# aniketntnu/WordDiffusion

Measured on AMD Instinct MI355X. Metric: denoised 64x256 word images/sec (1000-step DDPM), whole job, higher is better.
Workload: dtype bf16x3; 1 GPU; BASELINE configs[1]: batch 64 per GPU of 64x256 crops = [64,4,8,32] latents, 1000-step DDPM (999 executed steps), base unet.py UNetModel (320 ch, mult (1,1), 4 heads, 339 writers), random-init synthetic weights; variant=base, batch_per_gpu=64, noise_steps=1000, executed_steps_per_image=999, precision=split-bf16 MFMA x3, fp32 accumulate (<=1e-4 of the fp32 reference), output_finite=True

## Files before the change

include/wdiff_hip.h:

```cpp
#ifndef WDIFF_HIP_H
#define WDIFF_HIP_H

#include <stdint.h>

#ifdef __cplusplus
extern "C" {
#endif

#define WD_OK 0
#define WD_EINVAL (-1)
#define WD_ELAUNCH (-2)
#define WD_ESTATE (-3)

#define WD_ACT_NONE 0
#define WD_ACT_SILU 1
#define WD_ACT_GEGLU 2

typedef uint16_t wd_bf16;

#define WD_MAX_KSPLIT 64

typedef struct wd_src {
    const wd_bf16* hi;
    const wd_bf16* lo;
// ... 122 lines not shown
int wd_gemm_auto_ksplit(int m, int n, int ktot, int64_t ws_floats);
int wd_gemm_args_bytes(void);
int wd_gemm_experimental(void);

int wd_gn_nchunk(int hw);
int wd_gn_stats(const float* x, int ld, int batch, int hw, int c, int cpg, double* part, void* stream);
int wd_gn_fold_chunks(const double* part, int batch, int nchunk, int ngroups, double* out, void* stream);

int wd_gn_apply(const float* x, int ld, int batch, int hw, int c, int cpg, const double* part, int nchunk, int part_cpg,
                const float* gamma, const float* beta, float eps, int silu,
                wd_bf16* out_hi, wd_bf16* out_lo, int out_ld, int c_off,
                wd_bf16* raw_hi, wd_bf16* raw_lo, void* stream);

int wd_gn_apply2(const float* xa, int lda, int ca, const double* part_a, int nchunk_a, int part_cpg_a, int c_off_a,
                 const float* xb, int ldb, int cb, const double* part_b, int nchunk_b, int part_cpg_b, int c_off_b,
                 int batch, int hw, int cpg, const float* gamma, const float* beta, float eps, int silu,
                 wd_bf16* out_hi, wd_bf16* out_lo, int out_ld, wd_bf16* raw_hi, wd_bf16* raw_lo, const int32_t* perm_a, void* stream);

int wd_gn_conv3x3_few_supported(int c, int w, int oc);
int wd_gn_conv3x3_few(const float* x, int ld, int batch, int h, int w, int c, int cpg, const double* part, int nchunk, int part_cpg,
                      const float* gamma, const float* beta, float eps, int silu, const float* weight, const float* bias, int oc,
                      float* out, void* stream);

int wd_layernorm(const float* x, int ld, int rows, int c, const float* gamma, const float* beta, float eps,
                 wd_bf16* out_hi, wd_bf16* out_lo, int out_ld, void* stream);

int wd_split(const float* x, int ld, int rows, int c, int silu, wd_bf16* out_hi, wd_bf16* out_lo, int out_ld,
             void* stream);

int wd_attention(const float* q, int ldq, const float* k, int ldk, const float* v, int ldv,
                 int batch, int heads, int nq, int nk, int d, float scale,
                 float* out_f32, wd_bf16* out_hi, wd_bf16* out_lo, int out_ld, int out_rows, int out_row0,
                 void* stream);

int64_t wd_attention_packed_elems(int batch, int heads, int nk, int d);
int wd_attention_pack_kv(const float* k, int ldk, const float* v, int ldv, int batch, int heads, int nk, int d,
                         wd_bf16* img, void* stream);
int wd_attention_packed(const float* q, int ldq, const wd_bf16* img, int batch, int heads, int nq, int nk, int d,
                        float scale, float* out_f32, wd_bf16* out_hi, wd_bf16* out_lo, int out_ld, int out_rows,
                        int out_row0, void* stream);

int wd_timestep_embedding(const int64_t* t, int batch, const float* freqs, int half,
                          wd_bf16* out_hi, wd_bf16* out_lo, int out_ld, void* stream);

int wd_xattn_supported(int c, int heads, int L);
int wd_xattn_fold(const float* k, int ldk, const float* v, int ldv, int batch, int heads, int L, int d, float scale,
// ... 168 lines not shown
```

worddiffusion_amd/_native.py:

```python
from __future__ import annotations

import ctypes as C
import os
import re

_HERE = os.path.dirname(os.path.abspath(__file__))
LIB_PATH = os.environ.get("WDIFF_LIB") or os.path.join(_HERE, "libwdiff_hip.so")
HEADER_PATH = os.path.join(os.path.dirname(_HERE), "include", "wdiff_hip.h")

WD_OK, WD_EINVAL, WD_ELAUNCH, WD_ESTATE = 0, -1, -2, -3
ACT_NONE, ACT_SILU, ACT_GEGLU = 0, 1, 2
NCLASS = 13
CLASS_NAMES = ("gemm", "gn_stats", "gn_apply", "layernorm", "attention", "other", "gemm_other_tiles", "gemm_splitk_reduce",
               "gemm_two_per_cu", "gemm_weights_to_registers", "feed_forward_fused", "weight_gradient", "gemm_small_maps_whole_k")

_vp = C.c_void_p
_i = C.c_int
_f = C.c_float
_u64 = C.c_uint64


class WdSrc(C.Structure):
    _fields_ = [("hi", _vp), ("lo", _vp), ("gather", _vp), ("ld", C.c_int32), ("c", C.c_int32),
                ("ntaps", C.c_int32), ("hw_src", C.c_int32)]
# ... 42 lines not shown

_SIGS = {
    "wd_gemm": (_i, [C.POINTER(WdGemmArgs), _vp]),
    "wd_gemm_check": (_i, [C.POINTER(WdGemmArgs), C.POINTER(WdGemmArgs)]),
    "wd_dw": (_i, [C.POINTER(WdDwArgs), _vp]),
    "wd_dw_supported": (_i, [_i, _i, _i, _i, _i]),
    "wd_dw_slices": (_i, [_i, _i, _i, _i]),
    "wd_dw_args_bytes": (_i, []),
    "wd_dw_group": (_i, [C.POINTER(WdDwArgs), _vp, _vp, _i, _vp]),
    "wd_dw_group_slices": (_i, [_i, _i, _i, _i, _i]),
    "wd_dw_item_bytes": (_i, []),
    "wd_gemm_auto_ksplit": (_i, [_i, _i, _i, C.c_int64]),
    "wd_gemm_pack_w": (_i, [_vp, _vp, _i, _i, _vp, _vp, _vp]),
    "wd_ff_fused": (_i, [C.POINTER(WdFfArgs), _vp]),
    "wd_ff_supported": (_i, [_i, _i]),
    "wd_ff_args_bytes": (_i, []),
    "wd_gemm_args_bytes": (_i, []),
    "wd_gemm_experimental": (_i, []),
    "wd_gn_nchunk": (_i, [_i]),
    "wd_gn_stats": (_i, [_vp, _i, _i, _i, _i, _i, _vp, _vp]),
    "wd_gn_fold_chunks": (_i, [_vp, _i, _i, _i, _vp, _vp]),
    "wd_gn_conv3x3_few_supported": (_i, [_i, _i, _i]),
    "wd_gn_conv3x3_few": (_i, [_vp, _i, _i, _i, _i, _i, _i, _vp, _i, _i, _vp, _vp, _f, _i, _vp, _vp, _i, _vp, _vp]),
    "wd_gn_apply": (_i, [_vp, _i, _i, _i, _i, _i, _vp, _i, _i, _vp, _vp, _f, _i, _vp, _vp, _i, _i, _vp, _vp, _vp]),
    "wd_gn_apply2": (_i, [_vp, _i, _i, _vp, _i, _i, _i, _vp, _i, _i, _vp, _i, _i, _i, _i, _i, _i, _vp, _vp, _f, _i, _vp, _vp, _i, _vp,
                          _vp, _vp, _vp]),
    "wd_layernorm": (_i, [_vp, _i, _i, _i, _vp, _vp, _f, _vp, _vp, _i, _vp]),
    "wd_split": (_i, [_vp, _i, _i, _i, _i, _vp, _vp, _i, _vp]),
    "wd_attention": (_i, [_vp, _i, _vp, _i, _vp, _i, _i, _i, _i, _i, _i, _f, _vp, _vp, _vp, _i, _i, _i, _vp]),
    "wd_attention_packed_elems": (C.c_int64, [_i, _i, _i, _i]),
    "wd_attention_pack_kv": (_i, [_vp, _i, _vp, _i, _i, _i, _i, _i, _vp, _vp]),
    "wd_attention_packed": (_i, [_vp, _i, _vp, _i, _i, _i, _i, _i, _f, _vp, _vp, _vp, _i, _i, _i, _vp]),
    "wd_timestep_embedding": (_i, [_vp, _i, _vp, _i, _vp, _vp, _i, _vp]),
    "wd_embed_tokens": (_i, [_vp, _i, _i, _i, _vp, _i, _i, _vp, _vp, _vp, _i, _vp]),
    "wd_im2col3x3": (_i, [_vp, _i, _i, _i, _i, _vp, _vp, _i, _vp]),
    "wd_nchw_to_tokens": (_i, [_vp, _i, _i, _i, _vp, _i, _vp]),
    "wd_tokens_to_nchw": (_i, [_vp, _i, _i, _i, _i, _vp, _vp]),
    "wd_ddpm_step": (_i, [_vp, _vp, _i, _i, _vp, _vp, _vp, _vp, _vp, _u64, _u64, _vp]),
    "wd_advance_timestep": (_i, [_vp, _i, _vp, _i, _vp]),
    "wd_randn": (_i, [_vp, _i, _i, _u64, _u64, C.c_uint32, _vp]),
    "wd_noise_images": (_i, [_vp, _vp, _vp, _vp, _vp, _i, _i, _vp, _vp]),
    "wd_copy2d": (_i, [_vp, C.c_int64, _vp, C.c_int64, C.c_int64, C.c_int64, _vp]),
    "wd_ema_update": (_i, [_vp, _vp, C.c_int64, C.c_double, _vp]),
    "wd_adamw_table_entry_bytes": (_i, []),
    "wd_adamw_chunk": (_i, []),
    "wd_adamw_multi": (_i, [_vp, _i, C.c_int64, C.c_double, C.c_double, C.c_double, C.c_double, C.c_double, C.c_int64, _i,
# ... 100 lines not shown
```

worddiffusion_amd/csrc/wd_norm.hip:

```cpp
#include "wd_common.h"

namespace {

constexpr int GN_TOK = 32;

__global__ void gn_stats_kernel(const float* __restrict__ x, int ld, int hw, int c, int cpg, int nchunk,
                                double* __restrict__ part) {
    extern __shared__ __attribute__((aligned(16))) char smem[];
    float* s_sum = reinterpret_cast<float*>(smem);
    float* s_sq = s_sum + 2 * c;
    const int b = blockIdx.y, j = blockIdx.x;
    const int cx = threadIdx.x * 4;
    const int t0 = j * GN_TOK, t1 = min(hw, t0 + GN_TOK);
    if (cx < c) {
        float4 s = make_float4(0, 0, 0, 0), q = make_float4(0, 0, 0, 0);
        const float* base = x + ((long)b * hw) * ld + cx;
        for (int t = t0 + threadIdx.y; t < t1; t += 2) {
            const float4 v = *reinterpret_cast<const float4*>(base + (long)t * ld);
            s.x += v.x; s.y += v.y; s.z += v.z; s.w += v.w;
            q.x += v.x * v.x; q.y += v.y * v.y; q.z += v.z * v.z; q.w += v.w * v.w;
        }
        *reinterpret_cast<float4*>(s_sum + threadIdx.y * c + cx) = s;
        *reinterpret_cast<float4*>(s_sq + threadIdx.y * c + cx) = q;
    }
    __syncthreads();
    const int ng = c / cpg;
    const int tid = threadIdx.y * blockDim.x + threadIdx.x;
// ... 19 lines not shown
};

__global__ void gn_apply_kernel(const GnSrc s0, const GnSrc s1, int hw, int cpg, const float* __restrict__ gamma,
                                const float* __restrict__ beta, float eps, int silu, wd_bf16* __restrict__ out_hi,
                                wd_bf16* __restrict__ out_lo, int out_ld, wd_bf16* __restrict__ raw_hi,
                                wd_bf16* __restrict__ raw_lo) {
    const GnSrc& sr = blockIdx.z ? s1 : s0;
    const float* __restrict__ x = sr.x;
    const double* __restrict__ part = sr.part;
    const int ld = sr.ld, c = sr.c, nchunk = sr.nchunk, part_cpg = sr.part_cpg, c_off = sr.c_off;
    __shared__ float s_mean[32], s_rstd[32];
    const int b = blockIdx.y;
    const int ng = c / cpg;
    if (threadIdx.x < ng) {
        const int ratio = cpg / part_cpg, ngs = c / part_cpg;
        double ds = 0.0, dq = 0.0;
        for (int j = 0; j < nchunk; ++j) {
            const double* p = part + (((long)b * nchunk + j) * ngs + threadIdx.x * ratio) * 2;
            for (int k = 0; k < ratio; ++k) {
                ds += p[2 * k];
                dq += p[2 * k + 1];
            }
        }
        const double n = (double)hw * cpg;
        const double mean = ds / n;
        double var = dq / n - mean * mean;
        if (var < 0.0) var = 0.0;
        s_mean[threadIdx.x] = (float)mean;
        s_rstd[threadIdx.x] = (float)(1.0 / sqrt(var + (double)eps));
    }
    __syncthreads();
    const int c4 = c >> 2;
    const int t0 = blockIdx.x * AP_TOK, nt = min(AP_TOK, hw - t0);
    if (c4 <= 256) {
        const int rpp = 256 / c4;
        const int tl = threadIdx.x / c4, cx = (threadIdx.x - tl * c4) * 4;
        if (tl >= rpp) return;
        float sc[4], sh[4];
#pragma unroll
        for (int j = 0; j < 4; ++j) {
            const int g = (cx + j) / cpg;
            sc[j] = s_rstd[g] * gamma[c_off + cx + j];
            sh[j] = beta[c_off + cx + j] - s_mean[g] * sc[j];
        }
        for (int t = tl; t < nt; t += rpp) {
            const long row = (long)b * hw + t0 + t;
            const long srow = sr.perm ? (long)b * hw + sr.perm[t0 + t] : row;
            const float4 v = *reinterpret_cast<const float4*>(x + srow * ld + cx);
            float4 y = make_float4(v.x * sc[0] + sh[0], v.y * sc[1] + sh[1], v.z * sc[2] + sh[2], v.w * sc[3] + sh[3]);
            if (silu) {
                y.x = wd_silu(y.x); y.y = wd_silu(y.y); y.z = wd_silu(y.z); y.w = wd_silu(y.w);
            }
            uint2 h, l;
            wd_split4(y, h, l);
            const long o = row * out_ld + c_off + cx;
            *reinterpret_cast<uint2*>(out_hi + o) = h;
            if (out_lo) *reinterpret_cast<uint2*>(out_lo + o) = l;
            if (raw_hi) {
                wd_split4(v, h, l);
                *reinterpret_cast<uint2*>(raw_hi + o) = h;
                if (raw_lo) *reinterpret_cast<uint2*>(raw_lo + o) = l;
            }
        }
        return;
    }
    const int total = nt * c4;
    for (int i = threadIdx.x; i < total; i += blockDim.x) {
        const int t = i / c4, cx = (i - t * c4) * 4;
        const long row = (long)b * hw + t0 + t;
        const long srow = sr.perm ? (long)b * hw + sr.perm[t0 + t] : row;
        const float4 v = *reinterpret_cast<const float4*>(x + srow * ld + cx);
        float4 y;
        {
            const int g = cx / cpg, g1 = (cx + 1) / cpg, g2 = (cx + 2) / cpg, g3 = (cx + 3) / cpg;
            const float4 ga = *reinterpret_cast<const float4*>(gamma + c_off + cx);
// ... 204 lines not shown
    *reinterpret_cast<float4*>(s_red + ((long)cg * PXL + pl) * 4) = acc;
    __syncthreads();
    for (int i = tid; i < W * oc; i += 256) {
        const int o = i / W, px = i - o * W;
        float v = bias ? bias[o] : 0.f;
        for (int g = 0; g < CG; ++g) v += s_red[((long)g * PXL + px) * 4 + o];
        out[(((long)b * oc + o) * H + y) * W + px] = v;
    }
}

__global__ void __launch_bounds__(256) gn_fold_chunks_kernel(const double* __restrict__ part, int nchunk, int ng2,
                                                            double* __restrict__ out) {
    __shared__ double red[4][64];
    const int col = threadIdx.x & 63, lane = threadIdx.x >> 6;
    const long b = blockIdx.x;
    double acc = 0.0;
    if (col < ng2)
        for (int j = lane; j < nchunk; j += 4) acc += part[(b * nchunk + j) * ng2 + col];
    red[lane][col] = acc;
    __syncthreads();
    if (lane == 0 && col < ng2) out[b * ng2 + col] = (red[0][col] + red[1][col]) + (red[2][col] + red[3][col]);
}

}

extern "C" int wd_gn_nchunk(int hw) { return (hw + GN_TOK - 1) / GN_TOK; }

extern "C" int wd_gn_fold_chunks(const double* part, int batch, int nchunk, int ngroups, double* out, void* stream) {
    if (!part || !out || batch <= 0 || nchunk <= 0 || ngroups <= 0 || ngroups > 32) return WD_EINVAL;
    hipStream_t st = reinterpret_cast<hipStream_t>(stream);
    WdLaunchScope scope(WD_CLS_GNSTATS, st);
    hipLaunchKernelGGL(gn_fold_chunks_kernel, dim3(batch), dim3(256), 0, st, part, nchunk, 2 * ngroups, out);
    return wd_check_launch();
}

extern "C" int wd_gn_stats(const float* x, int ld, int batch, int hw, int c, int cpg, double* part, void* stream) {
    if (!x || !part || batch <= 0 || hw <= 0 || c <= 0 || cpg <= 0) return WD_EINVAL;
    if (c % 4 || ld % 4 || c % cpg || c / cpg > 256 || c > 4096) return WD_EINVAL;
    hipStream_t st = reinterpret_cast<hipStream_t>(stream);
    const int nchunk = wd_gn_nchunk(hw);
    const int bx = 64 * ((c / 4 + 63) / 64);
    if (bx * 2 > 1024) return WD_EINVAL;
    WdLaunchScope scope(WD_CLS_GNSTATS, st);
    hipLaunchKernelGGL(gn_stats_kernel, dim3(nchunk, batch), dim3(bx, 2), 4 * c * sizeof(float), st, x, ld, hw, c, cpg,
                       nchunk, part);
    return wd_check_launch();
// ... 35 lines not shown

extern "C" int wd_gn_conv3x3_few_supported(int c, int w, int oc) {
    return c > 0 && c % GC_CH == 0 && w > 0 && w <= 64 && oc >= 1 && oc <= 4 &&
           (size_t)(9 * GC_CH * 4 + gn_conv_tile_floats(w)) * sizeof(float) <= 64 * 1024;
}

extern "C" int wd_gn_conv3x3_few(const float* x, int ld, int batch, int h, int w, int c, int cpg, const double* part, int nchunk,
                                 int part_cpg, const float* gamma, const float* beta, float eps, int silu, const float* weight,
                                 const float* bias, int oc, float* out, void* stream) {
    if (!x || !part || !gamma || !beta || !weight || !out || batch <= 0 || h <= 0 || nchunk <= 0 || part_cpg <= 0) return WD_EINVAL;
    if (!wd_gn_conv3x3_few_supported(c, w, oc) || ld % 4 || cpg <= 0 || c % cpg || c / cpg > 32 || cpg % part_cpg) return WD_EINVAL;
    hipStream_t st = reinterpret_cast<hipStream_t>(stream);
    const size_t smem = (size_t)(9 * GC_CH * 4 + gn_conv_tile_floats(w)) * sizeof(float);
    WdLaunchScope scope(WD_CLS_OTHER, st);
    if (w <= 32)
        hipLaunchKernelGGL(gn_conv_few_kernel<32>, dim3(batch, h), dim3(256), smem, st, x, ld, h, w, c, cpg, nchunk, part_cpg, part,
                           gamma, beta, eps, silu, weight, bias, oc, out);
    else
        hipLaunchKernelGGL(gn_conv_few_kernel<64>, dim3(batch, h), dim3(256), smem, st, x, ld, h, w, c, cpg, nchunk, part_cpg, part,
                           gamma, beta, eps, silu, weight, bias, oc, out);
    return wd_check_launch();
}

extern "C" int wd_layernorm(const float* x, int ld, int rows, int c, const float* gamma, const float* beta, float eps,
                            wd_bf16* out_hi, wd_bf16* out_lo, int out_ld, void* stream) {
    if (!x || !gamma || !beta || !out_hi || rows <= 0 || c <= 0) return WD_EINVAL;
    if (c % 4 || ld % 4 || out_ld % 4 || c > 64 * 4 * LN_MAX4) return WD_EINVAL;
    hipStream_t st = reinterpret_cast<hipStream_t>(stream);
    WdLaunchScope scope(WD_CLS_LN, st);
    hipLaunchKernelGGL(layernorm_kernel, dim3((rows + 3) / 4), dim3(256), 0, st, x, ld, rows, c, gamma, beta, eps,
                       out_hi, out_lo, out_ld);
    return wd_check_launch();
}

extern "C" int wd_split(const float* x, int ld, int rows, int c, int silu, wd_bf16* out_hi, wd_bf16* out_lo, int out_ld,
                        void* stream) {
    if (!x || !out_hi || rows <= 0 || c <= 0 || c % 4 || ld % 4 || out_ld % 4) return WD_EINVAL;
    hipStream_t st = reinterpret_cast<hipStream_t>(stream);
    const long total = (long)rows * (c / 4);
    const int grid = (int)((total + 255) / 256 < 2048 ? (total + 255) / 256 : 2048);
    WdLaunchScope scope(WD_CLS_OTHER, st);
    hipLaunchKernelGGL(split_kernel, dim3(grid), dim3(256), 0, st, x, ld, rows, c, silu, out_hi, out_lo, out_ld);
    return wd_check_launch();
}
```

worddiffusion_amd/engine.py:

```python
from __future__ import annotations

import ctypes as C
import math
import os
from typing import Dict, List, Optional, Tuple

import numpy as np
import torch

from . import _native as N
from .layers import (DownsampleParams, ResBlockParams, SpatialTransformerParams, UpsampleParams)


def conv_gather_table(h: int, w: int, mode: str) -> Tuple[np.ndarray, int, int]:
    if mode == "same":
        ho, wo = h, w
    elif mode == "down":
        ho, wo = (h + 2 - 3) // 2 + 1, (w + 2 - 3) // 2 + 1
    elif mode == "up":
        ho, wo = 2 * h, 2 * w
    else:
        raise ValueError(mode)
    yy, xx = np.meshgrid(np.arange(ho), np.arange(wo), indexing="ij")
    tab = np.full((9, ho * wo), -1, dtype=np.int32)
# ... 192 lines not shown
                assert p.is_cuda and p.dtype == torch.float32 and p.is_contiguous(), name
                if mode == 2:
                    hi, lo, ld, ntc = d.data_ptr() + 4 * col_off, 0, 0, 1
                    nch = (n + vchunk - 1) // vchunk
                else:
                    ld = r.cols
                    o = 2 * (row_off * ld + col_off)
                    hi, lo = d[0].data_ptr() + o, d[1].data_ptr() + o
                    ntc = (c + tile - 1) // tile
                    nch = (((npad if mode == 1 else n) + tile - 1) // tile) * ntc
                recs.append(struct.pack("<QQQQiiiiiiiiqii", p.data_ptr(), p2.data_ptr() if p2 is not None else 0, hi, lo, n, c, t,
                                        mode, npad, ld, g, ntc, c0, 0, 0))
                c0 += nch
                if frag is not None and name in frag and self.frag_ok(r):
                    f = frag[name]
                    recs.append(struct.pack("<QQQQiiiiiiiiqii", p.data_ptr(), 0, f[0].data_ptr(), f[1].data_ptr(), n, c, t, 3, 0,
                                            r.rows, g, ntc, c0, row_off, col_off))
                    c0 += nch
        raw = torch.frombuffer(bytearray(b"".join(recs)), dtype=torch.uint8).to(dev)
        return raw, c0, len(recs)


class Act:
    __slots__ = ("t", "c", "h", "w", "stats", "prod", "perm")

    def __init__(self, t, c, h, w, stats=None, prod=None, perm=None):
        self.t, self.c, self.h, self.w = t, c, h, w
        self.perm = perm
        self.stats = stats
        self.prod = prod


class Plan:
    def __init__(self):
        self.cond: List[tuple] = []
        self.step: List[tuple] = []
        self.keep: List[object] = []
        self.out: Optional[torch.Tensor] = None

    @staticmethod
    def _run(ops, stream):
        for fn, args, what in ops:
            rc = fn(*args, stream)
            if rc != 0:
                N.check(rc, what)

    def run_cond(self, stream):
        self._run(self.cond, stream)

    def run_film(self, stream):
# ... 24 lines not shown
        self._pack = None
        self._w: Dict[str, torch.Tensor] = {}
        self._w3: Dict[str, torch.Tensor] = {}
        self._w3_meta: Dict[str, tuple] = {}
        self._wf: Dict[str, torch.Tensor] = {}
        self.use_wdirect = os.environ.get("WDIFF_GEMM_WDIRECT", "1") != "0"
        self.use_up_phases = os.environ.get("WDIFF_UPSAMPLE_PHASES", "1") != "0"
        self._derived: Dict[str, tuple] = {}
        self.use_smallmap = os.environ.get("WDIFF_GEMM_SMALLMAP", "1") != "0"
        self.fuse_ff = os.environ.get("WDIFF_FUSE_FF", "1") != "0"
        self.fuse_proj = os.environ.get("WDIFF_FUSE_PROJ", "1") != "0"
        self.fuse_ln = os.environ.get("WDIFF_FUSE_LN", "1") != "0"
        self.fuse_gn_in = int(os.environ.get("WDIFF_FUSE_GN_IN", "1"))
        self.use_slab = os.environ.get("WDIFF_SLAB", "0") != "0"
        self.fuse_stats = os.environ.get("WDIFF_FUSE_STATS", "1") != "0"
        self.fuse_xattn = os.environ.get("WDIFF_FUSE_XATTN", "1") != "0"
        self.use_conv3 = os.environ.get("WDIFF_CONV3", "0") != "0"
        if (self.use_slab or self.use_conv3) and not self.lib.wd_gemm_experimental():
            raise N.NativeError("WDIFF_SLAB / WDIFF_CONV3 need a library built with WDIFF_EXPERIMENTAL=1 "
                                "(python -m worddiffusion_amd.build --force)")
        self.fuse_xattn_pair = os.environ.get("WDIFF_FUSE_XATTN_PAIR", "1") != "0"
        self.fuse_st = os.environ.get("WDIFF_FUSE_ST", "1") != "0"
        self.fuse_out = os.environ.get("WDIFF_FUSE_OUT", "1") != "0"
        self.pack_kv = os.environ.get("WDIFF_PACK_KV", "1") != "0"
        self.fuse_gn2 = os.environ.get("WDIFF_FUSE_GN2", "1") != "0"
        self.fuse_gn = os.environ.get("WDIFF_FUSE_GN", "1") != "0"
        self.fuse_split = os.environ.get("WDIFF_FUSE_SPLIT", "1") != "0"
        self._plans: Dict[tuple, Plan] = {}
        self._tabs: Dict[tuple, torch.Tensor] = {}
        self._tab_np: Dict[int, np.ndarray] = {}
        self._same_w: Dict[int, int] = {}
        self._down_w: Dict[int, int] = {}
        self._ws = None
        self.device = None

    def set_precision(self, mode: str):
        npass = {"bf16x3": 3, "fp32": 3, "bf16": 1}[mode]
        if npass != self.npass:
            self.npass = npass
            self._plans.clear()

    def _recipes(self) -> "RecipeBook":
        m = self.model
        R = RecipeBook()
        film_w = []
        self.film_off = {}
        off = 0
        cin_conv = m.input_blocks[0][0]
        self.kpad_in = ((9 * cin_conv.in_channels + 31) // 32) * 32
        R.matrix("in.w", cin_conv.out_channels, self.kpad_in).fwd(cin_conv.weight)
        R.vector("in.b", cin_conv.bias)
        R.linear("te0", m.time_embed[0])
        R.linear("te2", m.time_embed[2])
        if m.num_classes is not None:
            R.vector("label", m.label_emb.weight)
        we = m.word_emb
        cd = we.embedding.weight.shape[1]
        R.vector("we.table", we.embedding.weight)
        qkv = (we.attention.linear_query, we.attention.linear_key, we.attention.linear_value)
        R.matrix("we.qkv.w", 3 * cd, cd)
        R.vector_cat("we.qkv.b", [l.bias for l in qkv])
        for i, l in enumerate(qkv):
            R["we.qkv.w"].fwd(l.weight, row_off=i * cd)
        kv_w = []
        self.kv_off = {}
        kvo = 0
        for name, mod in self._walk():
            if isinstance(mod, ResBlockParams):
                R.vector(name + ".gn1.g", mod.in_layers[0].weight)
                R.vector(name + ".gn1.b", mod.in_layers[0].bias)
                R.matrix(name + ".c1.w", mod.cout, 9 * mod.cin).fwd(mod.in_layers[2].weight)
                R.vector(name + ".c1.b", mod.in_layers[2].bias)
                R.vector(name + ".gn2.g", mod.out_layers[0].weight)
                R.vector(name + ".gn2.b", mod.out_layers[0].bias)
# ... 305 lines not shown
        if a32 is not None:
            self._set_a32(a, *a32)
        return self._legal(a, apply=False, **fields)

    def _give_tickets(self, a, m, n):
        ntick = ((m + 63) // 64) * ((n + 63) // 64)
        if ntick > 2048:
            return
        P = self._cur_plan
        tk = getattr(P, "_tickets", None)
        if tk is None or P._ticket_off + ntick > tk.numel():
            tk = torch.zeros(1 << 16, dtype=torch.int32, device=self.device)
            P.keep.append(tk)
            P._tickets, P._ticket_off = tk, 0
        a.tickets, a.ntickets = tk.data_ptr() + 4 * P._ticket_off, ntick
        P._ticket_off += ntick

    def _gn(self, P, ops, what, srcs: List[Act], gname, eps, silu, want_raw=False):
        B = self._B
        h, w = srcs[0].h, srcs[0].w
        hw = h * w
        ctot = sum(s.c for s in srcs)
        cpg = ctot // 32
        has_perm = any(s.perm is not None for s in srcs)
        if has_perm and not (len(srcs) == 2 and srcs[1].perm is None and self.fuse_gn2 and not any(s.c % cpg for s in srcs)):
            raise NotImplementedError(f"{what}: a phase-major map (Upsample) is read by the two-source GroupNorm of a decoder block only")
        if any(s.c % cpg for s in srcs):
            cat = self._f32(P, B * hw, ctot)
            coff = 0
            for s in srcs:
                ops.append((self.lib.wd_copy2d, (cat.data_ptr() + 4 * coff, 4 * ctot, s.t.data_ptr(), 4 * s.c, 4 * s.c,
                                                 B * hw), what + ":concat"))
                coff += s.c
            srcs = [Act(cat, ctot, h, w)]
        pl = self._planes(P, B * hw, ctot)
        raw = self._planes(P, B * hw, ctot) if want_raw else None
        for s in srcs:
            if s.stats is None:
                nchunk = self.lib.wd_gn_nchunk(hw)
                pc = s.c // 32
                part = torch.empty((B, nchunk, 32, 2), dtype=torch.float64, device=self.device)
                P.keep.append(part)
                ops.append((self.lib.wd_gn_stats, (s.t.data_ptr(), s.c, B, hw, s.c, pc, part.data_ptr()),
                            what + ":stats"))
                s.stats = (part, nchunk, pc)
        coff = 0
# ... 62 lines not shown
        if pr.out_f32 != s.t.data_ptr() or pr.out_hi or pr.gn_gamma or pr.n != s.c:
            return False
        return self._legal(pr, gn_gamma=gam.data_ptr() + 4 * coff, gn_beta=bet.data_ptr() + 4 * coff, gn_eps=float(eps),
                           gn_silu=int(silu), gn_cpg=cpg, out_hi=pl[0].data_ptr() + 2 * coff,
                           out_lo=(pl[1].data_ptr() + 2 * coff) if self.npass == 3 else None, out_pl_ld=pl.shape[2])

    def _ln(self, P, ops, what, x: torch.Tensor, rows, c, name):
        pl = self._planes(P, rows, c)
        ops.append((self.lib.wd_layernorm,
                    (x.data_ptr(), c, rows, c, self._w[name + ".g"].data_ptr(), self._w[name + ".b"].data_ptr(), 1e-5,
                     pl[0].data_ptr(), pl[1].data_ptr() if self.npass == 3 else None, c), what))
        return pl

    def _resblock(self, P, name, mod: ResBlockParams, srcs: List[Act]) -> Act:
        ops = P.step
        B = self._B
        h, w = srcs[0].h, srcs[0].w
        hw, M = h * w, B * h * w
        cin, cout = mod.cin, mod.cout
        assert cin == sum(s.c for s in srcs)
        tab, _, _ = self._table(h, w, "same")
        need_raw = cin != cout
        h1 = self._f32(P, M, cout)
        if self._gn_in_consumer(P, ops, name + ".gn1", srcs, need_raw, M, hw, cout, taps=9, gather=tab):
            s1, in1 = self._src32(srcs[0], 9, tab, hw), (srcs[0], name + ".gn1", 1e-5, True)
            raw = None
        else:
            a1, raw = self._gn(P, ops, name + ".gn1", srcs, name + ".gn1", 1e-5, True, want_raw=need_raw)
            s1, in1 = self._src(a1, cin, 9, tab, hw), None
        g1 = self._gemm(ops, name + ".conv1", [s1], name + ".c1.w", M, hw,
                        bias=self._w[name + ".c1.b"], rowvec=self._film.data_ptr() + 4 * self.film_off[name],
                        rowvec_ld=self.film_total, out_f32=h1, out_ld=cout, want_stats=True, a32=in1)
        h1a = Act(h1, cout, h, w, g1._stats, prod=g1)
        if self._gn_in_consumer(P, ops, name + ".gn2", [h1a], False, M, hw, cout, taps=9, gather=tab):
            s2, in2 = self._src32(h1a, 9, tab, hw), (h1a, name + ".gn2", 1e-5, True)
        else:
            a2, _ = self._gn(P, ops, name + ".gn2", [h1a], name + ".gn2", 1e-5, True)
            s2, in2 = self._src(a2, cout, 9, tab, hw), None
        out = self._f32(P, M, cout)
        if need_raw:
            g2 = self._gemm(ops, name + ".conv2+skip", [s2, self._src(raw, cin)],
                            name + ".c2.w", M, hw, bias=self._w[name + ".c2.b"], out_f32=out, out_ld=cout,
                            want_stats=True, a32=in2)
        else:
            g2 = self._gemm(ops, name + ".conv2", [s2], name + ".c2.w", M, hw,
                            bias=self._w[name + ".c2.b"], resid=srcs[0].t.data_ptr(), resid_ld=cout, out_f32=out,
                            out_ld=cout, want_stats=True, a32=in2)
# ... 326 lines not shown
                continue
            use_pe = (self.variant == "base") or (n_tok <= msl)
            if use_pe and n_tok > msl:
                raise ValueError(f"context length {n_tok} exceeds max_seq_len {msl} (the reference fails too)")
            e = self._planes(P, B * n_tok, cd)
            cond.append((lib.wd_embed_tokens,
                         (ids.data_ptr(), i64, B * n_tok, n_tok, self._w["we.table"].data_ptr(),
                          self._w["we.table"].shape[0], cd, self._w["pe"].data_ptr() if use_pe else None,
                          e[0].data_ptr(), e[1].data_ptr() if lo_ok else None, cd), "word_emb.embedding"))
            qkv = self._f32(P, B * n_tok, 3 * cd)
            self._gemm(cond, "word_emb.qkv", [self._src(e, cd)], "we.qkv.w", B * n_tok, n_tok,
                       bias=self._w["we.qkv.b"], out_f32=qkv, out_ld=3 * cd)
            self._attention(cond, "word_emb.attention", qkv.data_ptr(), 3 * cd, qkv.data_ptr() + 4 * cd, 3 * cd,
                            qkv.data_ptr() + 8 * cd, 3 * cd, 1, n_tok, n_tok, cd, 1.0, ctx_pl, out_rows=L,
                            out_row0=row0)
        P.ctx_pl = ctx_pl
        if self.kv_total:
            self._kv = self._f32(P, B * L, self.kv_total)
            self._gemm(cond, "cross.kv", [self._src(ctx_pl, cd)], "kv.w", B * L, L, out_f32=self._kv,
                       out_ld=self.kv_total)

        step = P.step
        has_lab = m.num_classes is not None
        self._film = self._f32(P, B, self.film_total)
        P.t_dev = torch.zeros((1,), dtype=torch.int32, device=dev)
        P.film = []
        if film_steps:
            T = film_steps
            chunk = min(T, max(8, FILM_CHUNK_ROWS // B))
            nchunks = (T + chunk - 1) // chunk
            Tp = nchunks * chunk
            film = P.film
            tt = torch.arange(Tp, dtype=torch.int64, device=dev)
            P.keep.append(tt)
            te = self._planes(P, Tp, mc)
            film.append((lib.wd_timestep_embedding, (tt.data_ptr(), Tp, self._w["freqs"].data_ptr(), mc // 2, te[0].data_ptr(),
                                                     te[1].data_ptr() if lo_ok else None, mc), "timestep_embedding[all t]"))
            e1 = self._planes(P, Tp, ted)
            self._gemm(film, "time_embed.0[all t]", [self._src(te, mc)], "te0.w", Tp, 1, bias=self._w["te0.b"], act=N.ACT_SILU,
                       out_pl=e1)
            tm = self._f32(P, Tp, ted)
            self._gemm(film, "time_embed.2[all t]", [self._src(e1, ted)], "te2.w", Tp, 1, bias=self._w["te2.b"], out_f32=tm,
                       out_ld=ted)
            e2 = self._planes(P, chunk * B, ted)
            P.film_table = self._f32(P, chunk * B, self.film_total)
            P.film_chunk, P.film_nchunks, P.film_loaded = chunk, nchunks, -1
            chunk_gemm = []
            self._gemm(chunk_gemm, "emb_layers(all)[chunk of t]", [self._src(e2, ted)], "film.w", chunk * B, 1,
                       bias=self._w["film.b"], out_f32=P.film_table, out_ld=self.film_total)
            lab = self._w["label"].data_ptr() if has_lab else None
            yin = P.y_in.data_ptr() if has_lab else None
            ncls = m.num_classes if has_lab else 0

            def film_prepare(t, stream, P=P, tm=tm, e2=e2, chunk=chunk, B=B):
                c = int(t) // chunk
                if c == P.film_loaded:
                    return False
                N.check(lib.wd_emb_combine(tm.data_ptr() + 4 * c * chunk * ted, lab, yin, ncls, chunk, B, ted, e2[0].data_ptr(),
                                           e2[1].data_ptr() if lo_ok else None, ted, stream), "SiLU(time + label)[chunk of t]")
                Plan._run(chunk_gemm, stream)
                P.film_loaded = c
                return True

            P.film_prepare = film_prepare
            step.append((lib.wd_select_rows, (P.film_table.data_ptr(), P.t_dev.data_ptr(), B, self.film_total, chunk,
                                              self._film.data_ptr()), "film rows of step t"))
        else:
            te = self._planes(P, B, mc)
            step.append((lib.wd_timestep_embedding, (P.t_in.data_ptr(), B, self._w["freqs"].data_ptr(), mc // 2,
                                                     te[0].data_ptr(), te[1].data_ptr() if lo_ok else None, mc),
                         "timestep_embedding"))
            e1 = self._planes(P, B, ted)
            self._gemm(step, "time_embed.0", [self._src(te, mc)], "te0.w", B, 1, bias=self._w["te0.b"], act=N.ACT_SILU,
                       out_pl=e1)
            e2 = self._planes(P, B, ted)
            self._gemm(step, "time_embed.2+label", [self._src(e1, ted)], "te2.w", B, 1, bias=self._w["te2.b"],
                       resid=self._w["label"].data_ptr() if has_lab else None, resid_ld=ted if has_lab else 0,
                       resid_rows=P.y_in.data_ptr() if has_lab else None, act=N.ACT_SILU, out_pl=e2)
            self._gemm(step, "emb_layers(all)", [self._src(e2, ted)], "film.w", B, 1, bias=self._w["film.b"],
                       out_f32=self._film, out_ld=self.film_total)

        xin = self._planes(P, B * H * W, self.kpad_in)
        step.append((lib.wd_im2col3x3, (P.x_in.data_ptr(), B, m.in_channels, H, W, xin[0].data_ptr(),
                                        xin[1].data_ptr() if lo_ok else None, self.kpad_in), "im2col"))
        h0 = self._f32(P, B * H * W, mc)
        g0 = self._gemm(step, "input_blocks.0", [self._src(xin, self.kpad_in)], "in.w", B * H * W, H * W,
                        bias=self._w["in.b"], out_f32=h0, out_ld=mc, want_stats=True)
        cur = Act(h0, mc, H, W, g0._stats)
        hs = [cur]

        def run_layers(prefix, blk, cur, extra=None):
            for j, mod in enumerate(blk):
                name = f"{prefix}.{j}"
                if isinstance(mod, ResBlockParams):
                    cur = self._resblock(P, name, mod, [cur] + ([extra] if (extra is not None and j == 0) else []))
                elif isinstance(mod, SpatialTransformerParams):
                    cur = self._transformer(P, name, mod, cur)
                elif isinstance(mod, DownsampleParams):
                    cur = self._resample(P, name, mod, cur, "down")
                elif isinstance(mod, UpsampleParams):
                    cur = self._resample(P, name, mod, cur, "up")
                else:
                    raise TypeError(type(mod))
            return cur

        for i, blk in enumerate(m.input_blocks):
            if i == 0:
                continue
            cur = run_layers(f"in{i}", blk, cur)
            hs.append(cur)
        cur = run_layers("mid", m.middle_block, cur)
# ... 78 lines not shown
```

Measured before the change: 34.87 images/s.

## Fuse input conv, first GroupNorm+SiLU and film row select into one head kernel

```diff
diff --git a/include/wdiff_hip.h b/include/wdiff_hip.h
--- a/include/wdiff_hip.h
+++ b/include/wdiff_hip.h
@@ -168,6 +168,12 @@
                       const float* gamma, const float* beta, float eps, int silu, const float* weight, const float* bias, int oc,
                       float* out, void* stream);
 
+int wd_in_conv_gn_supported(int cin, int h, int w, int cout, int cpg);
+int wd_in_conv_gn(const float* x, int batch, int cin, int h, int w, const float* weight, const float* bias, int cout,
+                  float* h0, int ld, double* part, int cpg, const float* gamma, const float* beta, float eps, int silu,
+                  wd_bf16* out_hi, wd_bf16* out_lo, int out_ld, const float* film_table, const int32_t* t_dev,
+                  int64_t row_floats, int chunk, float* film_out, void* stream);
+
 int wd_layernorm(const float* x, int ld, int rows, int c, const float* gamma, const float* beta, float eps,
                  wd_bf16* out_hi, wd_bf16* out_lo, int out_ld, void* stream);
 
diff --git a/worddiffusion_amd/_native.py b/worddiffusion_amd/_native.py
--- a/worddiffusion_amd/_native.py
+++ b/worddiffusion_amd/_native.py
@@ -88,6 +88,9 @@
     "wd_gn_fold_chunks": (_i, [_vp, _i, _i, _i, _vp, _vp]),
     "wd_gn_conv3x3_few_supported": (_i, [_i, _i, _i]),
     "wd_gn_conv3x3_few": (_i, [_vp, _i, _i, _i, _i, _i, _i, _vp, _i, _i, _vp, _vp, _f, _i, _vp, _vp, _i, _vp, _vp]),
+    "wd_in_conv_gn_supported": (_i, [_i, _i, _i, _i, _i]),
+    "wd_in_conv_gn": (_i, [_vp, _i, _i, _i, _i, _vp, _vp, _i, _vp, _i, _vp, _i, _vp, _vp, _f, _i, _vp, _vp, _i, _vp, _vp, C.c_int64, _i,
+                           _vp, _vp]),
     "wd_gn_apply": (_i, [_vp, _i, _i, _i, _i, _i, _vp, _i, _i, _vp, _vp, _f, _i, _vp, _vp, _i, _i, _vp, _vp, _vp]),
     "wd_gn_apply2": (_i, [_vp, _i, _i, _vp, _i, _i, _i, _vp, _i, _i, _vp, _i, _i, _i, _i, _i, _i, _vp, _vp, _f, _i, _vp, _vp, _i, _vp,
                           _vp, _vp, _vp]),
diff --git a/worddiffusion_amd/csrc/wd_norm.hip b/worddiffusion_amd/csrc/wd_norm.hip
--- a/worddiffusion_amd/csrc/wd_norm.hip
+++ b/worddiffusion_amd/csrc/wd_norm.hip
@@ -3,6 +3,25 @@
 namespace {
 
 constexpr int GN_TOK = 32;
+
+__device__ __forceinline__ void gn_mean_rstd(double ds, double dq, double n, float eps, float& mean_f, float& rstd_f) {
+    const double mean = ds / n;
+    double var = dq / n - mean * mean;
+    if (var < 0.0) var = 0.0;
+    mean_f = (float)mean;
+    rstd_f = (float)(1.0 / sqrt(var + (double)eps));
+}
+__device__ __forceinline__ void gn_scale_shift(float mean, float rstd, float gamma, float beta, float& sc, float& sh) {
+    sc = rstd * gamma;
+    sh = beta - mean * sc;
+}
+__device__ __forceinline__ float4 gn_affine4(const float4 v, const float* sc, const float* sh, int silu) {
+    float4 y = make_float4(v.x * sc[0] + sh[0], v.y * sc[1] + sh[1], v.z * sc[2] + sh[2], v.w * sc[3] + sh[3]);
+    if (silu) {
+        y.x = wd_silu(y.x); y.y = wd_silu(y.y); y.z = wd_silu(y.z); y.w = wd_silu(y.w);
+    }
+    return y;
+}
 
 __global__ void gn_stats_kernel(const float* __restrict__ x, int ld, int hw, int c, int cpg, int nchunk,
                                 double* __restrict__ part) {
@@ -68,12 +87,7 @@
                 dq += p[2 * k + 1];
             }
         }
-        const double n = (double)hw * cpg;
-        const double mean = ds / n;
-        double var = dq / n - mean * mean;
-        if (var < 0.0) var = 0.0;
-        s_mean[threadIdx.x] = (float)mean;
-        s_rstd[threadIdx.x] = (float)(1.0 / sqrt(var + (double)eps));
+        gn_mean_rstd(ds, dq, (double)hw * cpg, eps, s_mean[threadIdx.x], s_rstd[threadIdx.x]);
     }
     __syncthreads();
     const int c4 = c >> 2;
@@ -86,17 +100,13 @@
 #pragma unroll
         for (int j = 0; j < 4; ++j) {
             const int g = (cx + j) / cpg;
-            sc[j] = s_rstd[g] * gamma[c_off + cx + j];
-            sh[j] = beta[c_off + cx + j] - s_mean[g] * sc[j];
+            gn_scale_shift(s_mean[g], s_rstd[g], gamma[c_off + cx + j], beta[c_off + cx + j], sc[j], sh[j]);
         }
         for (int t = tl; t < nt; t += rpp) {
             const long row = (long)b * hw + t0 + t;
             const long srow = sr.perm ? (long)b * hw + sr.perm[t0 + t] : row;
             const float4 v = *reinterpret_cast<const float4*>(x + srow * ld + cx);
-            float4 y = make_float4(v.x * sc[0] + sh[0], v.y * sc[1] + sh[1], v.z * sc[2] + sh[2], v.w * sc[3] + sh[3]);
-            if (silu) {
-                y.x = wd_silu(y.x); y.y = wd_silu(y.y); y.z = wd_silu(y.z); y.w = wd_silu(y.w);
-            }
+            const float4 y = gn_affine4(v, sc, sh, silu);
             uint2 h, l;
             wd_split4(y, h, l);
             const long o = row * out_ld + c_off + cx;
@@ -347,6 +357,149 @@
     if (lane == 0 && col < ng2) out[b * ng2 + col] = (red[0][col] + red[1][col]) + (red[2][col] + red[3][col]);
 }
 
+typedef float wd_f2 __attribute__((ext_vector_type(2)));
+template <int CTRL>
+__device__ __forceinline__ double wd_dpp_f64(double v) {
+    return __hiloint2double(__builtin_amdgcn_update_dpp(0, __double2hiint(v), CTRL, 0xf, 0xf, true),
+                            __builtin_amdgcn_update_dpp(0, __double2loint(v), CTRL, 0xf, 0xf, true));
+}
+__device__ __forceinline__ double wd_readlane_f64(double v, int lane) {
+    return __hiloint2double(__builtin_amdgcn_readlane(__double2hiint(v), lane), __builtin_amdgcn_readlane(__double2loint(v), lane));
+}
+__device__ __forceinline__ double wd_wave_sum_f64(double v) {
+    v += wd_dpp_f64<0xB1>(v);
+    v += wd_dpp_f64<0x4E>(v);
+    v += wd_dpp_f64<0x124>(v);
+    v += wd_dpp_f64<0x128>(v);
+    return (wd_readlane_f64(v, 0) + wd_readlane_f64(v, 16)) + (wd_readlane_f64(v, 32) + wd_readlane_f64(v, 48));
+}
+template <int NCH>
+constexpr int ic_pitch() { return NCH + 4; }
+template <int NCH, int CIN, int SPLIT>
+__global__ void __launch_bounds__(256 * SPLIT) in_conv_gn_kernel(const float* __restrict__ x, int H, int W, const float* __restrict__ wgt,
+                                                        const float* __restrict__ bias, int cout, float* __restrict__ h0, int ld,
+                                                        double* __restrict__ part, int cpg, const float* __restrict__ gamma,
+                                                        const float* __restrict__ beta, float eps, int silu,
+                                                        wd_bf16* __restrict__ out_hi, wd_bf16* __restrict__ out_lo, int out_ld,
+                                                        const float* __restrict__ film_table, const int32_t* __restrict__ t_dev,
+                                                        long row4, int chunk, float* __restrict__ film_out) {
+    constexpr int K = 9 * CIN, PITCH = ic_pitch<NCH>(), Q = NCH / 4, NT = 256 * SPLIT, NCS = NCH / SPLIT;
+    static_assert(K % 2 == 0 && NCH % 4 == 0 && NCS % 2 == 0, "the multiply-adds run in pairs of taps and of channels, the stores in channel quads");
+    extern __shared__ __attribute__((aligned(16))) char smem[];
+    const int hw = H * W, Wp = W + 2, Hp = H + 2;
+    float* s_tile = reinterpret_cast<float*>(smem);
+    double* s_red = reinterpret_cast<double*>(s_tile + hw * PITCH);
+    float* s_sc = reinterpret_cast<float*>(s_red + 4 * NCH * 2);
+    float* s_sh = s_sc + NCH;
+    float* s_x = s_sh + NCH;
+    const int b = blockIdx.x, c0 = blockIdx.y * NCH, tid = threadIdx.x;
+    const int nx = CIN * Hp * Wp;
+    float hv[4];
+#pragma unroll
+    for (int k = 0; k < 4; ++k) {
+        const int i = tid + k * NT;
+        const int ci = i / (Hp * Wp), rem = i - ci * (Hp * Wp);
+        const int yy = rem / Wp - 1, xx = rem - (yy + 1) * Wp - 1;
+        hv[k] = (i < nx && yy >= 0 && yy < H && xx >= 0 && xx < W) ? x[(((long)b * CIN + ci) * H + yy) * W + xx] : 0.f;
+    }
+    const float ga = tid < NCH ? gamma[c0 + tid] : 0.f, be = tid < NCH ? beta[c0 + tid] : 0.f;
+    const long f_total = film_table ? (long)gridDim.x * row4 : 0, f_nthr = (long)gridDim.x * gridDim.y * NT;
+    const long f_base = film_table ? (long)((*t_dev) % chunk) * f_total : 0, f_i = ((long)blockIdx.y * gridDim.x + b) * NT + tid;
+    float4 fv = make_float4(0.f, 0.f, 0.f, 0.f);
+    if (f_i < f_total) fv = reinterpret_cast<const float4*>(film_table)[f_base + f_i];
+#pragma unroll
+    for (int k = 0; k < 4; ++k)
+        if (tid + k * NT < nx) s_x[tid + k * NT] = hv[k];
+    for (int i = tid + 4 * NT; i < nx; i += NT) {
+        const int ci = i / (Hp * Wp), rem = i - ci * (Hp * Wp);
+        const int yy = rem / Wp - 1, xx = rem - (yy + 1) * Wp - 1;
+        s_x[i] = (yy >= 0 && yy < H && xx >= 0 && xx < W) ? x[(((long)b * CIN + ci) * H + yy) * W + xx] : 0.f;
+    }
+    __syncthreads();
+    const int pos = tid & 255, sl = __builtin_amdgcn_readfirstlane(tid >> 8);
+    const bool act = pos < hw;
+    const int py = act ? pos / W : 0, px = act ? pos - py * W : 0;
+    float xv[K];
+#pragma unroll
+    for (int ci = 0; ci < CIN; ++ci)
+#pragma unroll
+        for (int dy = 0; dy < 3; ++dy)
+#pragma unroll
+            for (int dx = 0; dx < 3; ++dx) xv[ci * 9 + dy * 3 + dx] = s_x[(ci * Hp + py + dy) * Wp + px + dx];
+    const float* __restrict__ wb = wgt + (long)c0 * K;
+    double s = 0.0, q = 0.0;
+    int cnt = 0, g = sl * NCS / cpg;
+#pragma unroll 1
+    for (int j0 = sl * NCS; j0 < (sl + 1) * NCS; j0 += 2) {
+        float acc[2];
+#pragma unroll
+        for (int j = 0; j < 2; ++j) {
+            wd_f2 a = {0.f, 0.f};
+#pragma unroll
+            for (int k = 0; k < K; k += 2) {
+                const wd_f2 xx = {xv[k], xv[k + 1]}, ww = {wb[(j0 + j) * K + k], wb[(j0 + j) * K + k + 1]};
+                a = xx * ww + a;
+            }
+            acc[j] = (a.x + a.y) + (bias ? bias[c0 + j0 + j] : 0.f);
+        }
+        if (act) *reinterpret_cast<float2*>(s_tile + pos * PITCH + j0) = make_float2(acc[0], acc[1]);
+#pragma unroll
+        for (int j = 0; j < 2; ++j) {
+            const double v = act ? (double)acc[j] : 0.0;
+            s += v;
+            q += v * v;
+            if (++cnt == cpg) {
+                s = wd_wave_sum_f64(s);
+                q = wd_wave_sum_f64(q);
+                if ((tid & 63) == 0) *reinterpret_cast<double2*>(s_red + (((tid >> 6) & 3) * NCH + g) * 2) = make_double2(s, q);
+                ++g;
+                cnt = 0;
+                s = q = 0.0;
+            }
+        }
+    }
+    __syncthreads();
+    for (int i = tid; i < hw * Q; i += NT) {
+        const int r = i / Q, c4 = (i - r * Q) * 4;
+        *reinterpret_cast<float4*>(h0 + ((long)b * hw + r) * ld + c0 + c4) = *reinterpret_cast<const float4*>(s_tile + r * PITCH + c4);
+    }
+    if (f_i < f_total) reinterpret_cast<float4*>(film_out)[f_i] = fv;
+    for (long i = f_i + f_nthr; i < f_total; i += f_nthr)
+        reinterpret_cast<float4*>(film_out)[i] = reinterpret_cast<const float4*>(film_table)[f_base + i];
+    if (tid < NCH) {
+        const int g = tid / cpg;
+        const double2 r0 = *reinterpret_cast<const double2*>(s_red + (0 * NCH + g) * 2), r1 = *reinterpret_cast<const double2*>(s_red + (1 * NCH + g) * 2);
+        const double2 r2 = *reinterpret_cast<const double2*>(s_red + (2 * NCH + g) * 2), r3 = *reinterpret_cast<const double2*>(s_red + (3 * NCH + g) * 2);
+        const double ds = (r0.x + r1.x) + (r2.x + r3.x), dq = (r0.y + r1.y) + (r2.y + r3.y);
+        if (tid - g * cpg == 0) *reinterpret_cast<double2*>(part + ((long)b * (cout / cpg) + c0 / cpg + g) * 2) = make_double2(ds, dq);
+        float mean, rstd;
+        gn_mean_rstd(ds, dq, (double)hw * cpg, eps, mean, rstd);
+        gn_scale_shift(mean, rstd, ga, be, s_sc[tid], s_sh[tid]);
+    }
+    __syncthreads();
+    for (int i = tid; i < hw * Q; i += NT) {
+        const int r = i / Q, c4 = (i - r * Q) * 4;
+        const float4 v = *reinterpret_cast<const float4*>(s_tile + r * PITCH + c4);
+        const long row = (long)b * hw + r;
+        const float4 y = gn_affine4(v, s_sc + c4, s_sh + c4, silu);
+        uint2 h, l;
+        wd_split4(y, h, l);
+        const long o = row * out_ld + c0 + c4;
+        *reinterpret_cast<uint2*>(out_hi + o) = h;
+        if (out_lo) *reinterpret_cast<uint2*>(out_lo + o) = l;
+    }
+}
+template <int NCH>
+static size_t ic_smem(int cin, int h, int w) {
+    return (size_t)h * w * ic_pitch<NCH>() * 4 + 4 * NCH * 2 * 8 + 2 * NCH * 4 + (size_t)cin * (h + 2) * (w + 2) * 4;
+}
+static int ic_block(int cout, int cpg) {
+    if (cpg <= 0 || cout <= 0 || cout % cpg) return 0;
+    if (cout % 40 == 0 && 20 % cpg == 0) return 40;
+    if (cout % 32 == 0 && 16 % cpg == 0) return 32;
+    return 0;
+}
+
 }
 
 extern "C" int wd_gn_nchunk(int hw) { return (hw + GN_TOK - 1) / GN_TOK; }
@@ -428,6 +581,34 @@
     return wd_check_launch();
 }
 
+extern "C" int wd_in_conv_gn_supported(int cin, int h, int w, int cout, int cpg) {
+    if (cin != 4 || h <= 0 || w <= 0 || (long)h * w > 256) return 0;
+    const int nch = ic_block(cout, cpg);
+    if (!nch) return 0;
+    return (nch == 40 ? ic_smem<40>(cin, h, w) : ic_smem<32>(cin, h, w)) <= 64 * 1024;
+}
+
+extern "C" int wd_in_conv_gn(const float* x, int batch, int cin, int h, int w, const float* weight, const float* bias, int cout,
+                             float* h0, int ld, double* part, int cpg, const float* gamma, const float* beta, float eps, int silu,
+                             wd_bf16* out_hi, wd_bf16* out_lo, int out_ld, const float* film_table, const int32_t* t_dev,
+                             int64_t row_floats, int chunk, float* film_out, void* stream) {
+    if (!x || !weight || !h0 || !part || !gamma || !beta || !out_hi || batch <= 0) return WD_EINVAL;
+    if (!wd_in_conv_gn_supported(cin, h, w, cout, cpg) || ld % 4 || ld < cout || out_ld % 4 || out_ld < cout) return WD_EINVAL;
+    if (film_table && (!t_dev || !film_out || row_floats <= 0 || row_floats % 4 || chunk <= 0)) return WD_EINVAL;
+    hipStream_t st = reinterpret_cast<hipStream_t>(stream);
+    const int nch = ic_block(cout, cpg);
+    WdLaunchScope scope(WD_CLS_OTHER, st);
+    if (nch == 40)
+        hipLaunchKernelGGL((in_conv_gn_kernel<40, 4, 2>), dim3(batch, cout / 40), dim3(512), ic_smem<40>(cin, h, w), st, x, h, w, weight,
+                           bias, cout, h0, ld, part, cpg, gamma, beta, eps, silu, out_hi, out_lo, out_ld, film_table, t_dev,
+                           (long)(row_floats / 4), chunk, film_out);
+    else
+        hipLaunchKernelGGL((in_conv_gn_kernel<32, 4, 2>), dim3(batch, cout / 32), dim3(512), ic_smem<32>(cin, h, w), st, x, h, w, weight,
+                           bias, cout, h0, ld, part, cpg, gamma, beta, eps, silu, out_hi, out_lo, out_ld, film_table, t_dev,
+                           (long)(row_floats / 4), chunk, film_out);
+    return wd_check_launch();
+}
+
 extern "C" int wd_layernorm(const float* x, int ld, int rows, int c, const float* gamma, const float* beta, float eps,
                             wd_bf16* out_hi, wd_bf16* out_lo, int out_ld, void* stream) {
     if (!x || !gamma || !beta || !out_hi || rows <= 0 || c <= 0) return WD_EINVAL;
diff --git a/worddiffusion_amd/engine.py b/worddiffusion_amd/engine.py
--- a/worddiffusion_amd/engine.py
+++ b/worddiffusion_amd/engine.py
@@ -238,10 +238,11 @@
 
 
 class Act:
-    __slots__ = ("t", "c", "h", "w", "stats", "prod", "perm")
-
-    def __init__(self, t, c, h, w, stats=None, prod=None, perm=None):
+    __slots__ = ("t", "c", "h", "w", "stats", "prod", "perm", "normed")
+
+    def __init__(self, t, c, h, w, stats=None, prod=None, perm=None, normed=None):
         self.t, self.c, self.h, self.w = t, c, h, w
+        self.normed = normed
         self.perm = perm
         self.stats = stats
         self.prod = prod
@@ -312,6 +313,7 @@
         self.fuse_xattn_pair = os.environ.get("WDIFF_FUSE_XATTN_PAIR", "1") != "0"
         self.fuse_st = os.environ.get("WDIFF_FUSE_ST", "1") != "0"
         self.fuse_out = os.environ.get("WDIFF_FUSE_OUT", "1") != "0"
+        self.fuse_head = os.environ.get("WDIFF_FUSE_HEAD", "1") != "0"
         self.pack_kv = os.environ.get("WDIFF_PACK_KV", "1") != "0"
         self.fuse_gn2 = os.environ.get("WDIFF_FUSE_GN2", "1") != "0"
         self.fuse_gn = os.environ.get("WDIFF_FUSE_GN", "1") != "0"
@@ -340,6 +342,7 @@
         self.kpad_in = ((9 * cin_conv.in_channels + 31) // 32) * 32
         R.matrix("in.w", cin_conv.out_channels, self.kpad_in).fwd(cin_conv.weight)
         R.vector("in.b", cin_conv.bias)
+        R.vector("in.w.f32", cin_conv.weight)
         R.linear("te0", m.time_embed[0])
         R.linear("te2", m.time_embed[2])
         if m.num_classes is not None:
@@ -691,6 +694,8 @@
         hw = h * w
         ctot = sum(s.c for s in srcs)
         cpg = ctot // 32
+        if len(srcs) == 1 and srcs[0].normed is not None and srcs[0].normed[:3] == (gname, eps, bool(silu)) and not want_raw:
+            return srcs[0].normed[3], None
         has_perm = any(s.perm is not None for s in srcs)
         if has_perm and not (len(srcs) == 2 and srcs[1].perm is None and self.fuse_gn2 and not any(s.c % cpg for s in srcs)):
             raise NotImplementedError(f"{what}: a phase-major map (Upsample) is read by the two-source GroupNorm of a decoder block only")
@@ -799,7 +804,8 @@
         tab, _, _ = self._table(h, w, "same")
         need_raw = cin != cout
         h1 = self._f32(P, M, cout)
-        if self._gn_in_consumer(P, ops, name + ".gn1", srcs, need_raw, M, hw, cout, taps=9, gather=tab):
+        head_done = len(srcs) == 1 and srcs[0].normed is not None and srcs[0].normed[0] == name + ".gn1" and not need_raw
+        if not head_done and self._gn_in_consumer(P, ops, name + ".gn1", srcs, need_raw, M, hw, cout, taps=9, gather=tab):
             s1, in1 = self._src32(srcs[0], 9, tab, hw), (srcs[0], name + ".gn1", 1e-5, True)
             raw = None
         else:
@@ -1172,6 +1178,9 @@
 
         step = P.step
         has_lab = m.num_classes is not None
+        first = m.input_blocks[1][0] if len(m.input_blocks) > 1 and len(m.input_blocks[1]) else None
+        head = bool(self.fuse_head and isinstance(first, ResBlockParams) and first.cin == mc and first.cout == mc and mc % 32 == 0
+                    and lib.wd_in_conv_gn_supported(m.in_channels, H, W, mc, mc // 32))
         self._film = self._f32(P, B, self.film_total)
         P.t_dev = torch.zeros((1,), dtype=torch.int32, device=dev)
         P.film = []
@@ -1213,8 +1222,9 @@
                 return True
 
             P.film_prepare = film_prepare
-            step.append((lib.wd_select_rows, (P.film_table.data_ptr(), P.t_dev.data_ptr(), B, self.film_total, chunk,
-                                              self._film.data_ptr()), "film rows of step t"))
+            if not head:
+                step.append((lib.wd_select_rows, (P.film_table.data_ptr(), P.t_dev.data_ptr(), B, self.film_total, chunk,
+                                                  self._film.data_ptr()), "film rows of step t"))
         else:
             te = self._planes(P, B, mc)
             step.append((lib.wd_timestep_embedding, (P.t_in.data_ptr(), B, self._w["freqs"].data_ptr(), mc // 2,
@@ -1230,13 +1240,26 @@
             self._gemm(step, "emb_layers(all)", [self._src(e2, ted)], "film.w", B, 1, bias=self._w["film.b"],
                        out_f32=self._film, out_ld=self.film_total)
 
-        xin = self._planes(P, B * H * W, self.kpad_in)
-        step.append((lib.wd_im2col3x3, (P.x_in.data_ptr(), B, m.in_channels, H, W, xin[0].data_ptr(),
-                                        xin[1].data_ptr() if lo_ok else None, self.kpad_in), "im2col"))
         h0 = self._f32(P, B * H * W, mc)
-        g0 = self._gemm(step, "input_blocks.0", [self._src(xin, self.kpad_in)], "in.w", B * H * W, H * W,
-                        bias=self._w["in.b"], out_f32=h0, out_ld=mc, want_stats=True)
-        cur = Act(h0, mc, H, W, g0._stats)
+        if head:
+            part = torch.empty((B, 1, 32, 2), dtype=torch.float64, device=dev)
+            P.keep.append(part)
+            pl = self._planes(P, B * H * W, mc)
+            tbl = (P.film_table.data_ptr(), P.t_dev.data_ptr(), self.film_total, P.film_chunk, self._film.data_ptr()) if film_steps \
+                else (None, None, 0, 0, None)
+            step.append((lib.wd_in_conv_gn,
+                         (P.x_in.data_ptr(), B, m.in_channels, H, W, self._w["in.w.f32"].data_ptr(), self._w["in.b"].data_ptr(), mc,
+                          h0.data_ptr(), mc, part.data_ptr(), mc // 32, self._w["in1.0.gn1.g"].data_ptr(),
+                          self._w["in1.0.gn1.b"].data_ptr(), 1e-5, 1, pl[0].data_ptr(), pl[1].data_ptr() if lo_ok else None, mc) + tbl,
+                         "head: input_blocks.0 + in1.0.gn1" + (" + film rows of step t" if film_steps else "")))
+            cur = Act(h0, mc, H, W, (part, 1, mc // 32), normed=("in1.0.gn1", 1e-5, True, pl))
+        else:
+            xin = self._planes(P, B * H * W, self.kpad_in)
+            step.append((lib.wd_im2col3x3, (P.x_in.data_ptr(), B, m.in_channels, H, W, xin[0].data_ptr(),
+                                            xin[1].data_ptr() if lo_ok else None, self.kpad_in), "im2col"))
+            g0 = self._gemm(step, "input_blocks.0", [self._src(xin, self.kpad_in)], "in.w", B * H * W, H * W,
+                            bias=self._w["in.b"], out_f32=h0, out_ld=mc, want_stats=True)
+            cur = Act(h0, mc, H, W, g0._stats)
         hs = [cur]
 
         def run_layers(prefix, blk, cur, extra=None):
```

Result: faster. 35.33 images/s, median of 6 (+1.3%).
